# DerrickWang005/CRIS.pytorch

Hardware: AMD Instinct MI355X
Metric: train-step samples/sec, CRIS-R50 416x416 bs=64; loss parity vs ref (higher is better)
Workload: dtype bf16; 1 GPU; CRIS-R50 bf16 training step (fwd+BCE+bwd+Adam), 416x416, per-GPU bs=8, 17-token text, synthetic RefCOCO-shape batch resident in HBM (BASELINE.json configs[1]); global_batch=8, parallelism=dp1, launch=graph, graph_captured=True, syncbn_exchange=none, grad_exchange=none

## Files before the change

### cris/pytorch_amd/csrc/api.hip

```cpp
#include "common.h"
#include "../../../include/cris_hip.h"
#include <stdarg.h>
#include <string.h>

static thread_local char g_err[512] = {0};

void cris_set_error(const char* fmt, ...) {
    va_list ap;
    va_start(ap, fmt);
    vsnprintf(g_err, sizeof(g_err), fmt, ap);
    va_end(ap);
}

extern "C" const char* cris_last_error(void) { return g_err; }
extern "C" int cris_abi_version(void) { return CRIS_ABI_VERSION; }

extern "C" int cris_sizeof(const char* name) {
#define S(n) if (!strcmp(name, #n)) return (int)sizeof(n)
    S(cris_conv_gemm_params);
    S(cris_wgrad_params);
    S(cris_conv_gemm_group);
    S(cris_wgrad_group);
    S(cris_pack_desc);
    S(cris_conv_gemm_fp8_params);
    S(cris_pack_fp8_desc);
    S(cris_bn_apply_params);
    S(cris_bn_bwd_params);
    S(cris_ln_fwd_params);
    S(cris_ln_bwd_params);
    S(cris_sum_entry);
    S(cris_sum_group);
    S(cris_attn_params);
    S(cris_adam_desc);
    S(cris_ema_desc);
    S(cris_p2p_params);
    S(cris_p2p_link);
    S(cris_p2p_arena_params);
    S(cris_zero_ranges);
    S(cris_sample_desc);
    S(cris_eval_desc);
    S(cris_jpeg_info);
    S(cris_jpeg_image);
#undef S
    return -1;
}

extern "C" long cris_echo_conv_gemm(const void* vp) {
    const cris_conv_gemm_params* p = (const cris_conv_gemm_params*)vp;
    long h = 0;
    h = h * 31 + (long)(uintptr_t)p->A; h = h * 31 + (long)(uintptr_t)p->outT; h = h * 31 + p->T_sec_stride;
    h = h * 31 + p->lda; h = h * 31 + p->C; h = h * 31 + p->pad; h = h * 31 + p->ldb; h = h * 31 + p->K;
    h = h * 31 + p->act; h = h * 31 + p->out_f32; h = h * 31 + p->T_E; h = h * 31 + (long)(p->drop_p * 1000.f);
    h = h * 31 + p->drop_seed; h = h * 31 + p->drop_stream;
// ... 17 lines not shown
    const size_t tail0 = nvec * 16;
    if (blockIdx.x == 0 && tail0 + threadIdx.x < z.nbytes) reinterpret_cast<unsigned char*>(z.p)[tail0 + threadIdx.x] = 0;
}
extern "C" int cris_zero_many(const cris_zero_ranges* r, void* stream) {
    CRIS_CHECK_ARG(r && r->n > 0 && r->n <= CRIS_ZERO_RANGES_MAX, "1 .. CRIS_ZERO_RANGES_MAX ranges");
    size_t big = 0;
    for (int i = 0; i < r->n; ++i) {
        CRIS_CHECK_ARG(r->r[i].p && ((uintptr_t)r->r[i].p & 15) == 0, "ranges must be 16-byte aligned");
        if (r->r[i].nbytes > big) big = r->r[i].nbytes;
    }
    hipLaunchKernelGGL(zero_ranges_kernel, dim3(cris_grid_1d((long)(big / 16 + 1), 256, 2048), r->n), dim3(256), 0, (hipStream_t)stream, *r);
    CRIS_LAUNCH_CHECK();
    return 0;
}

extern "C" int cris_zero_bytes(void* p, size_t nbytes, void* stream) {
    if (!p || nbytes == 0) return 0;
    CRIS_CHECK_ARG(((uintptr_t)p & 15) == 0, "buffer must be 16-byte aligned");
    const size_t nvec = nbytes / 16;
    hipLaunchKernelGGL(zero_bytes_kernel, dim3(cris_grid_1d((long)(nvec ? nvec : 1), 256, 4096)), dim3(256), 0, (hipStream_t)stream,
                       (unsigned char*)p, nvec, nbytes);
    CRIS_LAUNCH_CHECK();
    return 0;
}
```

### cris/pytorch_amd/csrc/elementwise.hip

```cpp
#include <cmath>
#include "common.h"
#include "../../../include/cris_hip.h"

__device__ __forceinline__ void ld8f(const float* p, float* f) {
    const float4 a = *reinterpret_cast<const float4*>(p);
    const float4 b = *reinterpret_cast<const float4*>(p + 4);
    f[0] = a.x; f[1] = a.y; f[2] = a.z; f[3] = a.w; f[4] = b.x; f[5] = b.y; f[6] = b.z; f[7] = b.w;
}
__device__ __forceinline__ void ld8bf(const bf16_t* p, float* f) { unpack8(*reinterpret_cast<const uint4*>(p), f); }
__device__ __forceinline__ void st8bf(bf16_t* p, const float* f) { *reinterpret_cast<uint4*>(p) = pack8(f); }

#define GRID_STRIDE(idx, total) \
    for (long idx = (long)blockIdx.x * blockDim.x + threadIdx.x; idx < (total); idx += (long)gridDim.x * blockDim.x)

__global__ void stem_im2col_kernel(const float* __restrict__ img, int Bn, int H, int W, int OH, int OW, bf16_t* __restrict__ out) {
    const long total = (long)Bn * OH * OW * 4;
    const bool small = total < (1L << 24);
    GRID_STRIDE(idx, total) {
        const cris_idx4 q = cris_split4(idx, 4, OW, OH, small);
        const int kc = q.cv, ow = q.x, oh = q.y, b = q.b;
        const long m = idx >> 2;
        float v[8];
#pragma unroll
        for (int j = 0; j < 8; ++j) {
// ... 478 lines not shown
            float a = 0.f;
            for (int b = 0; b < Bn; ++b) a += dx[((size_t)b * L + r) * D + d];
            dpos[(size_t)r * D + d] = a;
        }
    }
}
extern "C" int cris_embed_bwd(const int64_t* tokens, const float* dx, int Bn, int L, int D, float* dtable, float* dpos,
                              unsigned char* row_live, void* stream) {
    CRIS_CHECK_ARG(tokens && dx && dtable && dpos, "bad args");
    hipLaunchKernelGGL(embed_bwd_kernel, dim3(cris_grid_1d((long)Bn * L * D, 256)), dim3(256), 0, (hipStream_t)stream, tokens, dx,
                       Bn, L, D, dtable, dpos, row_live);
    CRIS_LAUNCH_CHECK();
    return 0;
}

__global__ void eot_gather_kernel(const int64_t* tokens, const bf16_t* x, int L, int D, bf16_t* out, int* eot_index) {
    __shared__ int s_idx;
    const int b = blockIdx.x;
    if (threadIdx.x == 0) {
        int best = 0;
        int64_t bv = tokens[(size_t)b * L];
        for (int l = 1; l < L; ++l) {
            const int64_t v = tokens[(size_t)b * L + l];
            if (v > bv) { bv = v; best = l; }
        }
        s_idx = best;
        eot_index[b] = best;
    }
    __syncthreads();
    const bf16_t* src = x + ((size_t)b * L + s_idx) * D;
// ... 414 lines not shown
    CRIS_LAUNCH_CHECK();
    return 0;
}
extern "C" int cris_seg_loss_bwd(const float* logits, const float* target, int Bn, int HW, float w_bce, float w_dice, float pw, float s,
                                 const float* coef, const float* gscale, float* dlogits, void* stream) {
    CRIS_CHECK_ARG(logits && target && coef && dlogits, "null operand");
    CRIS_CHECK_ARG(Bn >= 1, "Bn must be >= 1");
    CRIS_CHECK_ARG(HW >= 1, "HW must be >= 1");
    if (seg_loss_check_config(__func__, w_bce, w_dice, pw, s)) return -1;
    hipLaunchKernelGGL(seg_loss_bwd_kernel, dim3(cris_grid_1d(HW, 256, 1024), Bn < SEG_MAX_GRID_Y ? Bn : SEG_MAX_GRID_Y), dim3(256), 0,
                       (hipStream_t)stream, logits, target, Bn, HW, w_bce, w_dice, pw, coef, gscale, dlogits);
    CRIS_LAUNCH_CHECK();
    return 0;
}

__global__ __launch_bounds__(1024) void train_metric_kernel(const float* x, const float* t, int Bn, int HW, float thr, float pr_iou, float* out) {
    __shared__ float si[16], su[16];
    float iou_sum = 0.f, pr_sum = 0.f;
    for (int b = 0; b < Bn; ++b) {
        float inter = 0.f, uni = 0.f;
        for (int i = threadIdx.x; i < HW; i += 1024) {
            const bool o = 1.f / (1.f + __expf(-x[(size_t)b * HW + i])) >= thr;
            const bool g = t[(size_t)b * HW + i] != 0.f;
            inter += (o && g) ? 1.f : 0.f;
            uni += (o || g) ? 1.f : 0.f;
        }
        inter = wave_sum(inter);
        uni = wave_sum(uni);
        __syncthreads();
        if ((threadIdx.x & 63) == 0) { si[threadIdx.x >> 6] = inter; su[threadIdx.x >> 6] = uni; }
        __syncthreads();
        if (threadIdx.x == 0) {
            float a = 0.f, u = 0.f;
#pragma unroll
            for (int w = 0; w < 16; ++w) { a += si[w]; u += su[w]; }
            const float iou = a / (u + 1e-6f);
            iou_sum += iou;
            pr_sum += iou > pr_iou ? 1.f : 0.f;
        }
    }
    if (threadIdx.x == 0) {
        out[0] = 100.f * iou_sum / (float)Bn;
        out[1] = 100.f * pr_sum / (float)Bn;
    }
}
extern "C" int cris_train_metric(const float* logits, const float* target, int Bn, int HW, float thr, float pr_iou, float* out,
                                 void* stream) {
    CRIS_CHECK_ARG(logits && target && out, "bad args");
    hipLaunchKernelGGL(train_metric_kernel, dim3(1), dim3(1024), 0, (hipStream_t)stream, logits, target, Bn, HW, thr, pr_iou, out);
    CRIS_LAUNCH_CHECK();
    return 0;
}

#define ADAM_ELEMS 8192
#define AP_T 64
#define AP_TN(PT) ((PT) == 9 ? 32 : 64)
#define AP_LROW(PT) (AP_T * (PT) + 2)

struct adam_coef {
    float beta1, beta2, eps, wd, bc1, rsb2, gscale;
    float keep;
};
__device__ __forceinline__ float adam_mul_rn(float a, float b) {
#pragma clang fp contract(off)
// ... 302 lines not shown
```

### cris/pytorch_amd/engine.py

```python
from __future__ import annotations

from typing import Callable, Dict, List, Optional

import torch
from torch import nn

from . import debug, ops, tables
from .arch import ClipSpec, HeadSpec, build_param_tree
from .ops import BF16, Drop, Geom, NO_DROP, pad8, pad32

F32 = torch.float32
BN_EPS, BN_MOM, LN_EPS = 1e-5, 0.1, 1e-5


class Act:
    __slots__ = ("t", "Bn", "H", "W", "C", "ld", "coff", "root", "_g", "aux")
    _engine = None

    def __init__(self, t, Bn, H, W, C, ld=None, coff=0, root=None):
        self.t, self.Bn, self.H, self.W, self.C = t, Bn, H, W, C
        self.ld = ld if ld is not None else C
        self.coff = coff
        self.root = root if root is not None else self
        self._g = None
# ... 62 lines not shown
        self.state_f32 = os.environ.get("CRIS_STATE_FP32", "0") == "1"
        self.P, self.Bf = params, buffers
        self.comm = comm or Comm()
        self.sync_bn = sync_bn and (self.comm.world > 1 or debug.HOOKS.force_dist)
        self.tape: List[Callable[[], None]] = []
        self.training = True
        self.seed = 0
        self.seed_dev = None
        self.loss_spec = None
        self.loss_terms = None
        self.side = torch.cuda.Stream(device=device) if torch.device(device).type == "cuda" else None
        if debug.HOOKS.no_side_stream:
            self.side = None
        self._wq, self._sq = ops.WgradQueue(self._flush_wgrads), ops.SumQueue()
        self._zslab, self._zcur, self._zneed, self._zneed_last = None, 0, 0, 0
        self._tables = {}
        self._build_grad_arena()
        self._build_packs()

    def gemm_layout(self, name):
        p = self.P[name]
        if name == "backbone.visual.conv1.weight":
            return p.shape[0], 27, 1, 32
        if p.dim() == 4:
            return p.shape[0], p.shape[1], p.shape[2] * p.shape[3], pad8(p.shape[1])
        return None

    def grad_param_layout(self, name):
        g, lay = self.G[name], self.gemm_layout(name)
        if lay is None or (lay[2] == 1 and lay[3] == lay[1]):
# ... 71 lines not shown
        self.grad_arena = torch.zeros(total, dtype=F32, device=self.dev)
        self.G = {name: self.grad_arena[o:o + n].view(shapes[name]) for name, (o, n) in offs.items()}
        self.grad_order = order
        self.grad_offsets = offs
        self.bn_pairs = pairs
        self.stage_ranges, zr = {}, {}
        for name in order:
            st = stage(name)
            lo, hi = offs[name][0], offs[name][0] + (offs[name][1] + 3) // 4 * 4
            a, b = self.stage_ranges.get(st, (lo, hi))
            self.stage_ranges[st] = (min(a, lo), max(b, hi))
            if needs_zero(name):
                a, b = zr.get(st, (lo, hi))
                zr[st] = (min(a, lo), max(b, hi))
        self.zero_ranges = [self.grad_arena[a:b] for a, b in sorted(zr.values())]

    def _add_pack(self, name, N, Cin, taps, Cpad=None, want_D=True, transposed=False):
        src = self.P[name]
        tab = self.packs[self.stage_of(name)]
        f, d = tab.add(src, N, Cin, taps, Cpad=Cpad, want_D=want_D, src_transposed=transposed)
        self.WF[name], self.WD[name] = f, d
        self.pack_info[name] = tab.info[-1]

    def _build_packs(self):
        self.packs = {st: ops.PackTable() for st in range(8)}
        self.packs_current = False
        self.WF, self.WD, self.pack_info = {}, {}, {}
        wd = not self.inference_only
        for name, p in self.P.items():
            if p.dim() == 4:
# ... 14 lines not shown
    def repack_stage(self, st):
        self.packs[st].run()

    def table(self, key, fn):
        if key not in self._tables:
            self._tables[key] = torch.from_numpy(fn()).to(self.dev)
        return self._tables[key]

    def _zero_slab_begin(self):
        need = self._zneed_last
        if need and (self._zslab is None or self._zslab.numel() < need):
            self._zslab = torch.empty(need, dtype=torch.uint8, device=self.dev)
        if self._zslab is not None:
            ops.zero_(self._zslab)
        self._zcur = self._zneed = 0

    def zeros(self, *shape, dtype=F32):
        n = dtype.itemsize
        for d in shape:
            n *= int(d)
        n_al = (n + 255) // 256 * 256
        self._zneed += n_al
        if n > 0 and self._zslab is not None and self._zcur + n_al <= self._zslab.numel():
            t = self._zslab[self._zcur:self._zcur + n].view(dtype).view(*shape)
            self._zcur += n_al
            return t
        return ops.zero_(torch.empty(*shape, dtype=dtype, device=self.dev))

    def empty(self, *shape, dtype=BF16):
        return torch.empty(*shape, dtype=dtype, device=self.dev)
# ... 208 lines not shown
                    dx, accum = dx_stream.grad_target()
                else:
                    dx, acc = x.grad_target()
                    accum = False
                    assert not acc, "bf16 LN input gradient cannot be accumulated"
                ops.ln_bwd(x.t, gamma, mean, rstd, rows, C, dx, ldx=x.ld, dy=None if (y is None or y.g is None) else y.g,
                           dypos=None if (ypos is None or ypos.g is None) else ypos.g,
                           dout_f32=None if outs is None else outs.g, dgamma=self.G[pfx + ".weight"], dbeta=self.G[pfx + ".bias"],
                           dx_accum=accum, in_relu=in_relu, in_drop=in_drop, out_drop=out_drop, queue=self._sq)

            self.tape.append(bwd)
        return y, ypos, outs

    def new_T(self, B, Hn, L, secs=1):
        Lpad = pad32(L)
        buf = self.zeros(secs, B * Hn * 64, Lpad, dtype=BF16)
        return dict(buf=buf, L=L, Lpad=Lpad, E=Hn * 64, sec_stride=B * Hn * 64 * Lpad)

    def attention(self, q: Act, k: Act, v: Act, Qt, Kt, Vt, B, Hn, Lq, Lk, *, causal=False, key_tokens=None, drop: Drop = NO_DROP):
        E = Hn * 64
        o = self.new_act(B, Lq, 1, E)
        lse = self.empty(B * Hn, Lq, dtype=F32)
        Lkp, Lqp = pad32(Lk), pad32(Lq)
        qv, kv, vv = q.t[:, q.coff:], k.t[:, k.coff:], v.t[:, v.coff:]
        prm = ops.attn_params(qv, kv, vv, Vt, B, Hn, Lq, Lk, Lkp, 64 ** -0.5, ldq=q.ld, ldk=k.ld, ldv=v.ld, Kt=Kt, Qt=Qt,
                              Lq_pad=Lqp, key_tokens=key_tokens, causal=causal, drop=drop)
        ops.attn_fwd(prm, o.t, lse, ldo=o.ld)
        if self.training:
            dOt = self.new_T(B, Hn, Lq)
            keep = (qv, kv, vv, Qt, Kt, Vt, key_tokens)

# ... 139 lines not shown
        if self.state_f32 and B <= ops.SMALL_MAX_ROWS:
            state = self._state_f32(word, x, xf, eot, B, L, D)
        else:
            rows = Act(self.empty(B, D), B, 1, 1, D)
            ops.eot_gather(word, xf.t, D, rows.t, eot)
            if self.training:
                def bwd_eot():
                    gx, acc = xf.grad_target()
                    if not acc:
                        ops.zero_(gx)
                    ops.eot_scatter_add(eot, rows.g, B, L, D, gx)
                self.tape.append(bwd_eot)
            state = self.gemm(rows, "backbone.text_projection", self.clip.embed_dim, w_transposed=True)
        if self.training:
            def bwd_embed():
                ops.embed_bwd(word, x0.g, self.G["backbone.token_embedding.weight"], self.G["backbone.positional_embedding"],
                              row_live=self.embed_live)
            self.tape.insert(self._text_tape_start, bwd_embed)
        return xf, state

    def _state_f32(self, word, x: Act, xf: Act, eot, B, L, D) -> Act:
        E = self.clip.embed_dim
        mean, rstd = xf.aux["ln_stats"]
        Pn = "backbone.text_projection"
        rows = torch.empty(B, D, dtype=F32, device=self.dev)
        ops.eot_gather_ln_f32(word, x.t, mean, rstd, self.P["backbone.ln_final.weight"], self.P["backbone.ln_final.bias"], D, rows, eot)
        state = Act(torch.empty(B, E, dtype=F32, device=self.dev), B, 1, 1, E)
        ops.linear_f32_small(rows, self.P[Pn], state.t, w_is_kn=True)
        if self.training:
            def bwd():
# ... 326 lines not shown
                ops.seg_loss_bwd(pred, msk, spec, coef, self._gscale, dpred)
            gx, acc = x.grad_target()
            assert not acc
            self._dwb = self.zeros(B, wb.ld)
            ops.dynconv_bwd(x.t, dpred, B, OH, OW, c, wb.t, gx, self._dwb)

        self.tape.append(bwd_loss)
        return pred, msk, loss.view(())

    def backward(self, gscale: Optional[torch.Tensor] = None, on_stage_done: Optional[Callable[[int], None]] = None):
        self._gscale = gscale
        Act._engine = self
        if debug.HOOKS.zero_all:
            ops.zero_(self.grad_arena)
        else:
            ops.zero_ranges(self.zero_ranges)
        marks = dict(self._stage_marks)
        (t0, t1), (v0, v1) = self._ranges["text"], self._ranges["visual"]
        head_start = max(t1, v1)
        def fire(i):
            if i in marks:
                self._flush_queues()
                if on_stage_done is not None:
                    for st in marks[i]:
                        on_stage_done(st)

        for i in range(len(self.tape) - 1, head_start - 1, -1):
            self.tape[i]()
            fire(i)
        self._flush_queues()
        if debug.HOOKS.hold_backward_fork:
# ... 32 lines not shown
```

### cris/pytorch_amd/hip.py

```python
import contextlib
import ctypes as C
import os

import torch

_HERE = os.path.dirname(os.path.abspath(__file__))
LIB_PATH = os.path.join(_HERE, "csrc", "libcris_hip.so")
if os.environ.get("CRIS_LIB_VARIANT"):
    LIB_PATH = os.path.join(_HERE, "csrc", "variants", "libcris_hip_%s.so" % os.environ["CRIS_LIB_VARIANT"])

P, I, L, F, U = C.c_void_p, C.c_int, C.c_long, C.c_float, C.c_uint32


class ConvGemmParams(C.Structure):
    _fields_ = [("A", P), ("Wt", P), ("bias", P), ("resid", P), ("out", P), ("outT", P), ("colsum", P), ("colsq", P),
                ("T_sec_stride", L),
                ("lda", I), ("a_coff", I),
                ("Bn", I), ("H", I), ("W", I), ("C", I),
                ("OH", I), ("OW", I), ("KH", I), ("KW", I), ("stride", I), ("pad", I),
                ("ldb", I),
                ("M", I), ("N", I), ("K", I),
                ("act", I),
                ("ldr", I), ("r_coff", I), ("resid_f32", I),
                ("ldc", I), ("c_coff", I), ("out_f32", I),
# ... 161 lines not shown
class EmaDesc(C.Structure):
    _fields_ = [("p", P), ("ema", P), ("n", L), ("row_live", P), ("row_len", I), ("block_start", I)]


ZERO_RANGES_MAX = 16


class ZeroRange(C.Structure):
    _fields_ = [("p", P), ("nbytes", C.c_size_t)]


class ZeroRanges(C.Structure):
    _fields_ = [("n", I), ("pad_", I), ("r", ZeroRange * ZERO_RANGES_MAX)]


class SampleDesc(C.Structure):
    _fields_ = [("img", P), ("mask", P), ("H", I), ("W", I), ("inv", C.c_double * 6)]


class EvalDesc(C.Structure):
    _fields_ = [("m", C.c_double * 6), ("w_out", I), ("h_out", I), ("map", I), ("row", I),
                ("mask_off", L), ("out_off", L), ("pitch", I), ("pad_", I)]


class JpegInfo(C.Structure):
    _fields_ = [("width", I), ("height", I), ("ncomp", I), ("hmax", I), ("vmax", I), ("mcus_x", I), ("mcus_y", I),
                ("restart_interval", I),
                ("comp_h", I * 3), ("comp_v", I * 3), ("blocks_w", I * 3), ("blocks_h", I * 3), ("down_w", I * 3), ("down_h", I * 3),
                ("quant", (C.c_ushort * 64) * 3),
                ("coef_offset", L * 3), ("coef_count", L), ("plane_offset", L * 3), ("plane_bytes", L), ("scan_offset", L),
# ... 15 lines not shown

class P2PLink(C.Structure):
    _fields_ = [("boxes", P), ("err", P), ("gen_dev", P),
                ("gen_host", I), ("rank", I), ("world", I),
                ("slot", I), ("slots", I), ("max_floats", I), ("spin_limit", I)]


class P2PArenaParams(C.Structure):
    _fields_ = [("arenas", P), ("lo", C.c_long), ("n", C.c_long), ("link", P2PLink), ("blocks", I)]


STRUCTS = {
    "cris_conv_gemm_params": ConvGemmParams, "cris_conv_gemm_group": ConvGemmGroup, "cris_wgrad_params": WgradParams, "cris_wgrad_group": WgradGroup, "cris_pack_desc": PackDesc,
    "cris_conv_gemm_fp8_params": ConvGemmFp8Params, "cris_pack_fp8_desc": PackFp8Desc,
    "cris_bn_apply_params": BnApplyParams, "cris_bn_bwd_params": BnBwdParams, "cris_ln_fwd_params": LnFwdParams,
    "cris_ln_bwd_params": LnBwdParams, "cris_sum_entry": SumEntry, "cris_sum_group": SumGroup, "cris_attn_params": AttnParams, "cris_adam_desc": AdamDesc, "cris_ema_desc": EmaDesc, "cris_p2p_params": P2PParams, "cris_p2p_link": P2PLink, "cris_p2p_arena_params": P2PArenaParams, "cris_zero_ranges": ZeroRanges,
    "cris_sample_desc": SampleDesc, "cris_eval_desc": EvalDesc, "cris_jpeg_info": JpegInfo, "cris_jpeg_image": JpegImage,
}

_SIGS = {
    "cris_last_error": (C.c_char_p, []),
    "cris_abi_version": (I, []),
    "cris_sizeof": (I, [C.c_char_p]),
    "cris_echo_conv_gemm": (L, [P]),
    "cris_conv_gemm": (I, [P, P]),
    "cris_conv_wgrad": (I, [P, P]),
    "cris_conv_wgrad_group": (I, [P, P]),
    "cris_conv_wgrad_tile": (I, [P]),
    "cris_wgrad_reduce": (I, [P, P]),
    "cris_wgrad_reduce_group": (I, [P, P]),
    "cris_wgrad_ws_floats": (L, [I, I, I, I]),
# ... 41 lines not shown
    "cris_fill_coords": (I, [P, I, I, I, I, I, I, P]),
    "cris_gather_samples_bf16": (I, [P, I, I, P, I, I, I, P, I, I, P]),
    "cris_add_bf16": (I, [P, I, I, P, I, I, P, I, I, I, I, P]),
    "cris_add_rowtable": (I, [P, I, P, I, P, I, I, I, P]),
    "cris_cast_f32_bf16": (I, [P, P, L, P]),
    "cris_cast_bf16_f32": (I, [P, P, L, I, P]),
    "cris_cast_f32_bf16_drop": (I, [P, P, L, F, U, U, U, P, P]),
    "cris_step_advance": (I, [P, P, P, P]),
    "cris_step_advance_micro": (I, [P, P, P, I, I, P]),
    "cris_axpy_f32": (I, [P, P, F, L, P]),
    "cris_grad_accumulate": (I, [P, P, L, I, P]),
    "cris_quickgelu_fwd": (I, [P, P, L, P]),
    "cris_quickgelu_bwd": (I, [P, P, P, L, P]),
    "cris_embed_fwd": (I, [P, P, P, I, I, I, P, P]),
    "cris_embed_bwd": (I, [P, P, I, I, I, P, P, P, P]),
    "cris_eot_gather": (I, [P, P, I, I, I, P, P, P]),
    "cris_eot_scatter_add": (I, [P, P, I, I, I, P, P]),
    "cris_eot_gather_ln_f32": (I, [P, P, P, P, P, P, I, I, I, P, P, P]),
    "cris_eot_scatter_add_f32": (I, [P, P, I, I, I, P, P]),
    "cris_linear_f32_small": (I, [P, I, P, I, I, P, I, I, I, P, I, I, P]),
    "cris_outer_sum_f32_small": (I, [P, I, P, I, I, I, I, P, I, P, P]),
    "cris_colstats_f32_small": (I, [P, I, I, I, P, P, P]),
    "cris_bn_relu_f32_small": (I, [P, I, P, P, I, I, P, I, P]),
    "cris_bn_relu_bwd_reduce_f32_small": (I, [P, I, P, I, P, P, P, P, I, I, P, P]),
    "cris_bn_relu_bwd_apply_f32_small": (I, [P, I, P, I, P, P, P, P, P, F, I, I, P, I, P]),
    "cris_posresize_fwd": (I, [P, P, I, I, I, P, P]),
    "cris_posresize_bwd": (I, [P, P, I, I, I, P, P]),
    "cris_batch_rowsum": (I, [P, I, I, I, I, P, P]),
    "cris_dynconv_fwd": (I, [P, I, I, I, I, P, I, P, P]),
    "cris_dynconv_bwd": (I, [P, P, I, I, I, I, P, I, P, P, P, P]),
    "cris_dynconv_bwd_ws_floats": (L, [I, I, I, I]),
    "cris_mask_resize_nearest": (I, [P, I, I, I, I, I, P, P]),
    "cris_bce_fwd": (I, [P, P, L, P, P, P]),
    "cris_bce_ws_floats": (I, []),
    "cris_bce_bwd": (I, [P, P, L, P, P, P]),
    "cris_seg_loss_fwd": (I, [P, P, I, I, F, F, F, F, P, P, P, P, P]),
    "cris_seg_loss_ws_floats": (L, [I]),
    "cris_seg_loss_bwd": (I, [P, P, I, I, F, F, F, F, P, P, P, P]),
    "cris_train_metric": (I, [P, P, I, I, F, F, P, P]),
    "cris_sigmoid_bicubic_up": (I, [P, I, I, I, I, I, P, P]),
    "cris_warp_affine_cubic": (I, [P, I, I, P, I, I, F, P, P]),
    "cris_threshold_iou": (I, [P, P, L, F, P, P]),
    "cris_eval_desc_fill": (I, [P, P, I, I, I, L, I, L, I]),
    "cris_eval_iou_batch": (I, [P, I, I, I, P, P, I, P, C.c_size_t, F, F, P, I, P, C.c_size_t, P]),
    "cris_predict_masks_batch": (I, [P, I, I, I, P, P, I, F, F, P, I, P, C.c_size_t, P]),
    "cris_preprocess_batch": (I, [P, I, I, I, P, P, P, P, P, P, P, P]),
    "cris_gray_sum_batch": (I, [P, P, I, P, P]),
    "cris_preprocess_batch_aug": (I, [P, I, I, I, P, P, P, P, P, P, P, P, P, P, P, P]),
    "cris_invert_affine": (I, [P, P]),
    "cris_remap_tables_u8": (I, [P, P]),
    "cris_zero_bytes": (I, [P, C.c_size_t, P]),
    "cris_zero_many": (I, [P, P]),
    "cris_adam_step": (I, [P, I, I, F, F, F, F, F, F, F, P, I, P]),
    "cris_adam_step_amp": (I, [P, I, I, F, F, F, F, F, F, F, P, P, P, I, P]),
    "cris_adamw_step": (I, [P, I, I, F, F, F, P, I, F, F, F, P, P, P, I, P]),
    "cris_counter_advance_unless": (I, [P, P, P]),
    "cris_adam_blocks": (I, [P]),
    "cris_adam_block_elems": (I, []),
    "cris_unpack_grads": (I, [P, I, I, P]),
    "cris_grad_sumsq": (I, [P, I, I, P, P]),
    "cris_grad_clip_finalize": (I, [P, I, F, F, P, P]),
    "cris_ema_blocks": (I, [P]),
    "cris_ema_advance": (I, [P, I, F, I, P, P]),
    "cris_ema_update": (I, [P, I, I, P, P]),
    "cris_adam_schedule_lrs": (I, [P, I, P, P, P, I, I, P, P]),
    "cris_p2p_mailbox_bytes": (C.c_size_t, [I, I, I]),
    "cris_p2p_alloc": (I, [C.c_size_t, P]),
# ... 119 lines not shown
```

### cris/pytorch_amd/ops.py

```python
from __future__ import annotations

import ctypes as C
import math
import os
from dataclasses import dataclass
from typing import Optional

import torch

from . import hip
from .hip import ptr

BF16 = torch.bfloat16


def _stream():
    return torch.cuda.current_stream().cuda_stream


def pad8(n: int) -> int:
    return (n + 7) // 8 * 8


def pad32(n: int) -> int:
# ... 696 lines not shown

def quickgelu_bwd(x, dy, dx):
    hip.call("cris_quickgelu_bwd", ptr(x), ptr(dy), ptr(dx), x.numel(), _stream())


def embed_fwd(tokens, table, pos, out):
    Bn, L = tokens.shape
    hip.call("cris_embed_fwd", ptr(tokens), ptr(table), ptr(pos), Bn, L, table.shape[1], ptr(out), _stream())


def embed_bwd(tokens, dx, dtable, dpos, row_live=None):
    Bn, L = tokens.shape
    hip.call("cris_embed_bwd", ptr(tokens), ptr(dx), Bn, L, dtable.shape[1], ptr(dtable), ptr(dpos), ptr(row_live), _stream())


def eot_gather(tokens, x, D, out, eot_index):
    Bn, L = tokens.shape
    hip.call("cris_eot_gather", ptr(tokens), ptr(x), Bn, L, D, ptr(out), ptr(eot_index), _stream())


def eot_scatter_add(eot_index, drows, Bn, L, D, dx):
    hip.call("cris_eot_scatter_add", ptr(eot_index), ptr(drows), Bn, L, D, ptr(dx), _stream())


SMALL_MAX_ROWS = 16


def eot_gather_ln_f32(tokens, x, mean, rstd, gamma, beta, D, out, eot_index):
    Bn, L = tokens.shape
    hip.call("cris_eot_gather_ln_f32", ptr(tokens), ptr(x), ptr(mean), ptr(rstd), ptr(gamma), ptr(beta), Bn, L, D, ptr(out), ptr(eot_index),
# ... 120 lines not shown


def seg_loss_fwd(logits, target, spec: SegLoss, loss, terms, coef):
    Bn = logits.shape[0]
    ws = torch.empty(hip.load().cris_seg_loss_ws_floats(Bn), dtype=torch.float32, device=logits.device)
    hip.call("cris_seg_loss_fwd", ptr(logits), ptr(target), Bn, logits.numel() // Bn, *spec.scalars, ptr(loss), ptr(terms), ptr(coef),
             ptr(ws), _stream())


def seg_loss_bwd(logits, target, spec: SegLoss, coef, gscale, dlogits):
    Bn = logits.shape[0]
    hip.call("cris_seg_loss_bwd", ptr(logits), ptr(target), Bn, logits.numel() // Bn, *spec.scalars, ptr(coef), ptr(gscale), ptr(dlogits),
             _stream())


def train_metric(logits, target, Bn, HW, out, thr=0.35, pr_iou=0.5):
    hip.call("cris_train_metric", ptr(logits), ptr(target), Bn, HW, float(thr), float(pr_iou), ptr(out), _stream())


def zero_(t):
    hip.call("cris_zero_bytes", ptr(t), t.numel() * t.element_size(), _stream())
    return t


def zero_ranges(tensors):
    for i in range(0, len(tensors), hip.ZERO_RANGES_MAX):
        chunk = tensors[i:i + hip.ZERO_RANGES_MAX]
        zr = hip.ZeroRanges()
        zr.n = len(chunk)
        for j, t in enumerate(chunk):
            zr.r[j].p, zr.r[j].nbytes = ptr(t), t.numel() * t.element_size()
        hip.call("cris_zero_many", C.byref(zr), _stream())


def torch_op(fn):
    fn()
    rec = hip.RECORDER
    if rec is not None:
        s = torch.cuda.current_stream()

        def run():
            if torch.cuda.current_stream() == s:
                fn()
            else:
                with torch.cuda.stream(s):
                    fn()
        rec.cmds.append((run, None, "torch_op"))
# ... 371 lines not shown
```

### cris/pytorch_amd/trainer.py

```python
import contextlib
import os
from typing import Optional

import torch

from . import capture, debug, ops
from .arch import ClipSpec, HeadSpec
from .engine import Engine


def strip_ddp_prefix(sd):
    keys = list(sd.keys())
    if keys and all(k.startswith("module.") for k in keys):
        return {k[len("module."):]: v for k, v in sd.items()}
    return sd


def split_state_dict(sd, device):
    sd = strip_ddp_prefix(sd)
    params = {k: v.to(device).contiguous() for k, v in sd.items()
              if v.is_floating_point() and not k.endswith(("running_mean", "running_var"))}
    buffers = {k: v.to(device).contiguous() for k, v in sd.items() if k.endswith(("running_mean", "running_var"))}
    return params, buffers

# ... 49 lines not shown
            for t in list(e.P.values()) + list(e.Bf.values()):
                self.comm.broadcast(t, 0)
        self._checked_batch = None
        names = [n for n in e.grad_order if n != "backbone.logit_scale"]
        self.names = names
        self.group = {n: (0 if in_backbone_group(n) else 1) for n in names}
        self.base_lr, self.lr_multi = base_lr, lr_multi
        self.weight_decay, self.decoupled_weight_decay, self.no_decay = decay_cfg
        self._no_decay_names = self._exempt(no_decay, [(n, e.P[n]) for n in names])
        if ((self.comm.world == 1 or getattr(self.comm, "supports_max_u8", False)) and self.weight_decays[EMBEDDING] == 0.0
                and os.environ.get("CRIS_ADAM_ROW_SKIP", "1") == "1" and torch.device(device).type == "cuda"):
            e.embed_live = torch.zeros(e.P["backbone.token_embedding.weight"].shape[0], dtype=torch.uint8, device=device)
        self._build_adam([base_lr] * len(names))
        self._apply_weight_decay()
        self.metric = torch.zeros(2, device=device)
        self.step_dev = torch.zeros(1, dtype=torch.int32, device=device)
        self.seed_dev = torch.zeros(1, dtype=torch.int32, device=device)
        self.xgen_dev = torch.zeros(1, dtype=torch.int32, device=device)
        self.syncbn_exchange = "none" if not e.sync_bn else "collective"
        if (e.sync_bn and os.environ.get("CRIS_SYNCBN_P2P", "1") == "1"
                and torch.device(device).type == "cuda" and hasattr(self.comm, "enable_p2p")):
            cmax = max(e.P[pfx + ".weight"].numel() for pfx in e.bn_prefixes)
            why = self.comm.enable_p2p(slots=2 * len(e.bn_prefixes) + 8, max_floats=4 * cmax, gen_dev=self.xgen_dev)
            if why is None:
                fused = getattr(self.comm, "_fused", False)
                self.syncbn_exchange = "p2p mailboxes, exchanged inside the BatchNorm launches" if fused else "p2p mailboxes, one exchange kernel per BatchNorm"
            else:
                self.syncbn_exchange = "collective (mailboxes refused: %s)" % why
        self.grad_exchange = "none" if (self.comm.world == 1 and not debug.HOOKS.force_dist) else "rccl"
        if (os.environ.get("CRIS_GRAD_EXCHANGE", "rccl") == "p2p" and getattr(self.comm, "p2p", None) is not None
# ... 58 lines not shown
        return float(max_norm)

    def _invalidate(self):
        self._graph = self._cmds = None
        self._eager_steps = 0

    def set_accum_steps(self, accum_steps):
        self.accum_steps = checked_int("accum_steps", accum_steps, 1)
        if self.accum_steps > 1:
            if self._acc is None:
                self._acc = torch.empty_like(self.engine.grad_arena)
                self._loss_acc = torch.zeros((), device=self.device)
                self._metric_micro = torch.zeros(2, device=self.device)
        else:
            self._acc = self._loss_acc = self._metric_micro = None
        self._size_terms_acc()
        self._invalidate()

    def set_loss(self, spec):
        self.engine.set_loss(spec)
        self._size_terms_acc()
        self._invalidate()

    def _size_terms_acc(self):
        if self.engine.loss_spec is not None and self.accum_steps > 1:
            if self._terms_acc is None:
                self._terms_acc = torch.zeros(2, device=self.device)
        else:
            self._terms_acc = None

# ... 127 lines not shown
                ops.axpy_f32(self._loss_acc, loss, 1.0 / K)
                if self._terms_acc is not None:
                    ops.axpy_f32(self._terms_acc, e.loss_terms, 1.0 / K)
            self._metric(pred, msk)
            e.backward(on_stage_done=self._stage_hook(m))
        if self._exchanges():
            ops.torch_op(self.comm.wait_all)
        self._update(1.0 / (self.comm.world * K))
        return (loss if K == 1 else self._loss_acc), pred, msk

    def _exchanges(self):
        return self.comm.world > 1 or debug.HOOKS.force_dist

    def _metric(self, pred, msk):
        e, K = self.engine, self.accum_steps
        if e.side is not None:
            cur = torch.cuda.current_stream()
            ops.torch_op(lambda: e.side.wait_stream(cur))
        with (torch.cuda.stream(e.side) if e.side is not None else contextlib.nullcontext()):
            ops.train_metric(pred, msk, pred.shape[0], pred.shape[2] * pred.shape[3], self.metric if K == 1 else self._metric_micro)
            if K > 1:
                ops.axpy_f32(self.metric, self._metric_micro, 1.0 / K)

    def _stage_hook(self, m):
        e, K, exchange = self.engine, self.accum_steps, self._exchanges()
        if K == 1 and not exchange:
            return None
        last = m == K - 1

        def on_stage(st):
            lo, hi = e.stage_ranges[st]
            g = e.grad_arena[lo:hi]
            if K > 1:
                acc = self._acc[lo:hi]
                if not last:
# ... 172 lines not shown
```

### include/cris_hip.h

```cpp
#ifndef CRIS_HIP_H
#define CRIS_HIP_H
#include <stddef.h>
#include <stdint.h>
#ifdef __cplusplus
extern "C" {
#endif

typedef uint16_t cris_bf16;

const char* cris_last_error(void);
#define CRIS_ABI_VERSION 8
int cris_abi_version(void);
int cris_sizeof(const char* struct_name);
long cris_echo_conv_gemm(const void* conv_gemm_params);

typedef struct {
    const cris_bf16* A;
    const cris_bf16* Wt;
    const float* bias;
    const void* resid;
    void* out;
    cris_bf16* outT;
    float* colsum;
    float* colsq;
// ... 254 lines not shown
                      int C, void* stream);
int cris_cast_f32_bf16(const float* x, cris_bf16* y, long n, void* stream);
int cris_cast_bf16_f32(const cris_bf16* x, float* y, long n, int accum, void* stream);
int cris_cast_f32_bf16_drop(const float* x, cris_bf16* y, long n, float drop_p, uint32_t drop_thresh, uint32_t seed,
                            uint32_t stream_id, const uint32_t* seed_dev, void* stream);
int cris_step_advance(int32_t* step, uint32_t* seed, int32_t* exchange_gen, void* stream);
int cris_step_advance_micro(int32_t* step, uint32_t* seed, int32_t* exchange_gen, int micro, int accum, void* stream);
int cris_axpy_f32(float* dst, const float* src, float alpha, long n, void* stream);
int cris_grad_accumulate(float* dst, const float* src, long n, int mode, void* stream);
int cris_quickgelu_fwd(const cris_bf16* x, cris_bf16* y, long n, void* stream);
int cris_quickgelu_bwd(const cris_bf16* x, const cris_bf16* dy, cris_bf16* dx, long n, void* stream);
int cris_embed_fwd(const int64_t* tokens, const float* table, const float* pos, int Bn, int L, int D, float* out,
                   void* stream);
int cris_embed_bwd(const int64_t* tokens, const float* dx, int Bn, int L, int D, float* dtable, float* dpos, unsigned char* row_live,
                   void* stream);
int cris_eot_gather(const int64_t* tokens, const cris_bf16* x, int Bn, int L, int D, cris_bf16* out, int* eot_index,
                    void* stream);
int cris_eot_scatter_add(const int* eot_index, const cris_bf16* dstate_rows, int Bn, int L, int D, cris_bf16* dx,
                         void* stream);
int cris_posresize_fwd(const float* R, const float* pos, int T, int G, int C, float* posr, void* stream);
int cris_posresize_bwd(const float* R, const float* dposr, int T, int G, int C, float* dpos, void* stream);
int cris_batch_rowsum(const cris_bf16* dx, int ldx, int Bn, int T, int C, float* out, void* stream);
int cris_dynconv_fwd(const cris_bf16* x, int Bn, int H, int W, int C, const float* wb, int ldwb, float* pred,
                     void* stream);
int cris_dynconv_bwd(const cris_bf16* x, const float* dpred, int Bn, int H, int W, int C, const float* wb, int ldwb,
                     cris_bf16* dx, float* dwb, float* ws, void* stream);
long cris_dynconv_bwd_ws_floats(int Bn, int H, int W, int ldwb);
int cris_mask_resize_nearest(const float* mask, int Bn, int IH, int IW, int OH, int OW, float* out, void* stream);
int cris_bce_fwd(const float* logits, const float* target, long n, float* loss, float* ws, void* stream);
int cris_bce_ws_floats(void);
int cris_bce_bwd(const float* logits, const float* target, long n, const float* gscale, float* dlogits, void* stream);
int cris_seg_loss_fwd(const float* logits, const float* target, int Bn, int HW, float w_bce, float w_dice, float pw, float s,
                      float* loss, float* terms, float* coef, float* ws, void* stream);
long cris_seg_loss_ws_floats(int Bn);
int cris_seg_loss_bwd(const float* logits, const float* target, int Bn, int HW, float w_bce, float w_dice, float pw, float s,
                      const float* coef, const float* gscale, float* dlogits, void* stream);
int cris_train_metric(const float* logits, const float* target, int Bn, int HW, float thr, float pr_iou, float* out,
                      void* stream);
int cris_sigmoid_bicubic_up(const float* logits, int Bn, int h, int w, int H, int W, float* out, void* stream);
int cris_warp_affine_cubic(const float* src, int H, int W, const double* mat, int w_out, int h_out, float border, float* dst,
                           void* stream);
int cris_threshold_iou(const float* pred, const float* mask, long n, float thr, int* counts, void* stream);
typedef struct {
    double m[6];
    int w_out, h_out;
    int map, row;
    long mask_off, out_off;
    int pitch, pad_;
} cris_eval_desc;
int cris_eval_desc_fill(cris_eval_desc* desc, const double* mat, int w_out, int h_out, int map, long mask_off, int pitch,
                        long out_off, int row);
int cris_eval_iou_batch(const float* probs, int P, int H, int W, const cris_eval_desc* descs_host, const cris_eval_desc* descs_dev,
                        int n, const unsigned char* masks, size_t mask_bytes, float thr, float border, int* counts, int count_rows,
// ... 12 lines not shown
                          const float* lut_img, const float* lut_mask, const unsigned char* border_rgb ,
                          float* img_out, float* mask_out, void* stream);
int cris_gray_sum_batch(const cris_sample_desc* samples_host, const cris_sample_desc* samples_dev, int n, unsigned long long* sums_dev,
                        void* stream);
int cris_preprocess_batch_aug(const cris_sample_desc* samples_dev, int n, int S_h, int S_w, const short* tab_linear, const short* tab_cubic,
                              const float* lut_img, const float* lut_mask, const unsigned char* border_rgb ,
                              const float* factors_dev, const unsigned long long* sums_dev, const float* unit_dev,
                              const float* norm , float* img_out, float* mask_out, void* stream);
int cris_invert_affine(const double* mat, double* inv);
int cris_remap_tables_u8(short* tab_linear, short* tab_cubic);
int cris_zero_bytes(void* p, size_t nbytes, void* stream);
#define CRIS_ZERO_RANGES_MAX 16
typedef struct { void* p; size_t nbytes; } cris_zero_range;
typedef struct { int n; int pad_; cris_zero_range r[CRIS_ZERO_RANGES_MAX]; } cris_zero_ranges;
int cris_zero_many(const cris_zero_ranges* r, void* stream);

typedef struct {
    float* p; const float* g; float* m; float* v;
    long n;
    float lr; float pad_;
    int block_start; int taps;
    int cin; int cpad;
    cris_bf16* dstF; cris_bf16* dstD;
    int N; int npad;
    int transposed; int ldF;
    const unsigned char* row_live;
    int row_len; int ldD;
} cris_adam_desc;
int cris_adam_step(const cris_adam_desc* dev_table, int n_desc, int total_blocks, float beta1, float beta2, float eps,
                   float weight_decay, float bias_corr1, float bias_corr2, float grad_scale, const int32_t* step_dev,
// ... 139 lines not shown
```

Measured before the change: 681.6 samples/s.

## Skip dense zeroing of embedding grad, pool attention T buffers, parallelize train metric

Three separate changes cut redundant work in the training step. First, the token-embedding gradient table is dropped from the per-step dense zero ranges. Instead, only the rows touched by earlier steps are re-zeroed, using a ring of recorded token ids. Second, the padded attention transpose buffers are pooled across steps, and only their pad tail columns are zeroed rather than the whole slab. Third, the train-metric kernel moves from a single block to one block per sample, with a last-block atomic reduction. Together these remove bulk memset traffic and a serialized reduction, at the cost of stateful buffers whose correctness depends on the slot and ring logic.

```diff
diff --git a/cris/pytorch_amd/csrc/api.hip b/cris/pytorch_amd/csrc/api.hip
--- a/cris/pytorch_amd/csrc/api.hip
+++ b/cris/pytorch_amd/csrc/api.hip
@@ -37,6 +37,7 @@
     S(cris_p2p_link);
     S(cris_p2p_arena_params);
     S(cris_zero_ranges);
+    S(cris_zero_tails);
     S(cris_sample_desc);
     S(cris_eval_desc);
     S(cris_jpeg_info);
@@ -84,6 +85,45 @@
     return 0;
 }
 
+#define ZT_WORDS 1024
+__device__ __host__ static inline int zero_tail_words(const cris_zero_tail& z) { return z.rows * ((z.ld - (z.col0 & ~1)) >> 1); }
+__global__ __launch_bounds__(256) void zero_tails_kernel(const cris_zero_tails t) {
+    int blk = blockIdx.x, i = 0;
+    for (; i < t.n; ++i) {
+        const int nb = (zero_tail_words(t.t[i]) + ZT_WORDS - 1) / ZT_WORDS;
+        if (blk < nb) break;
+        blk -= nb;
+    }
+    if (i == t.n) return;
+    const cris_zero_tail z = t.t[i];
+    const int c0 = z.col0 & ~1;
+    const int nw = (z.ld - c0) >> 1, total = z.rows * nw;
+    for (int w = blk * ZT_WORDS + threadIdx.x; w < total && w < (blk + 1) * ZT_WORDS; w += 256) {
+        const int row = w / nw;
+        const int col = c0 + 2 * (w - row * nw);
+        unsigned short* q = reinterpret_cast<unsigned short*>(z.p) + (size_t)row * z.ld + col;
+        if (col < z.col0) q[1] = 0;
+        else *reinterpret_cast<unsigned*>(q) = 0u;
+    }
+}
+extern "C" int cris_zero_tails_bf16(const cris_zero_tails* t, void* stream) {
+    CRIS_CHECK_ARG(t && t->n > 0 && t->n <= CRIS_ZERO_TAILS_MAX, "1 .. CRIS_ZERO_TAILS_MAX matrices");
+    long blocks = 0;
+    for (int i = 0; i < t->n; ++i) {
+        const cris_zero_tail& z = t->t[i];
+        CRIS_CHECK_ARG(z.p && ((uintptr_t)z.p & 3) == 0, "matrices must be 4-byte aligned");
+        CRIS_CHECK_ARG(z.rows >= 1 && z.ld >= 2 && (z.ld & 1) == 0, "rows >= 1 and an even ld");
+        CRIS_CHECK_ARG(z.col0 >= 0 && z.col0 <= z.ld && z.ld - z.col0 <= CRIS_ZERO_TAIL_COLS, "col0 must be within CRIS_ZERO_TAIL_COLS of ld");
+        CRIS_CHECK_ARG(z.rows <= (1 << 26), "rows must be <= 2^26");
+        blocks += (zero_tail_words(z) + ZT_WORDS - 1) / ZT_WORDS;
+    }
+    if (blocks == 0) return 0;
+    CRIS_CHECK_ARG(blocks < (1L << 31), "too many rows");
+    hipLaunchKernelGGL(zero_tails_kernel, dim3((unsigned)blocks), dim3(256), 0, (hipStream_t)stream, *t);
+    CRIS_LAUNCH_CHECK();
+    return 0;
+}
+
 extern "C" int cris_zero_bytes(void* p, size_t nbytes, void* stream) {
     if (!p || nbytes == 0) return 0;
     CRIS_CHECK_ARG(((uintptr_t)p & 15) == 0, "buffer must be 16-byte aligned");
diff --git a/cris/pytorch_amd/csrc/elementwise.hip b/cris/pytorch_amd/csrc/elementwise.hip
--- a/cris/pytorch_amd/csrc/elementwise.hip
+++ b/cris/pytorch_amd/csrc/elementwise.hip
@@ -516,6 +516,30 @@
     return 0;
 }
 
+__global__ __launch_bounds__(1024) void embed_rezero_kernel(int64_t* ids, int n_slots, int cap, int slot, const int64_t* tokens, int R, int D,
+                                                            int vocab, float* dtable) {
+    const int DV = D >> 2, lane = threadIdx.x & 63;
+    for (int r = threadIdx.x >> 6; r < n_slots * cap; r += 16) {
+        const int64_t tok = ids[r];
+        if (tok < 0 || tok >= vocab) continue;
+        float4* row = reinterpret_cast<float4*>(dtable + (size_t)tok * D);
+        for (int dv = lane; dv < DV; dv += 64) row[dv] = make_float4(0.f, 0.f, 0.f, 0.f);
+    }
+    __syncthreads();
+    for (int r = threadIdx.x; r < cap; r += 1024) ids[(size_t)slot * cap + r] = r < R ? tokens[r] : -1;
+}
+extern "C" int cris_embed_rezero(int64_t* ids, int n_slots, int cap, int slot, const int64_t* tokens, int R, int D, int vocab,
+                                 float* dtable, void* stream) {
+    CRIS_CHECK_ARG(ids && tokens && dtable, "null operand");
+    CRIS_CHECK_ARG(n_slots >= 1 && slot >= 0 && slot < n_slots, "slot must be in [0, n_slots)");
+    CRIS_CHECK_ARG(R >= 1 && R <= cap, "R must be in [1, cap]");
+    CRIS_CHECK_ARG(D >= 4 && !(D & 3) && vocab >= 1, "D must be a multiple of 4, vocab >= 1");
+    CRIS_CHECK_ARG(((uintptr_t)dtable & 15) == 0, "dtable must be 16-byte aligned");
+    hipLaunchKernelGGL(embed_rezero_kernel, dim3(1), dim3(1024), 0, (hipStream_t)stream, ids, n_slots, cap, slot, tokens, R, D, vocab, dtable);
+    CRIS_LAUNCH_CHECK();
+    return 0;
+}
+
 __global__ void eot_gather_kernel(const int64_t* tokens, const bf16_t* x, int L, int D, bf16_t* out, int* eot_index) {
     __shared__ int s_idx;
     const int b = blockIdx.x;
@@ -960,10 +984,11 @@
     return 0;
 }
 
-__global__ __launch_bounds__(1024) void train_metric_kernel(const float* x, const float* t, int Bn, int HW, float thr, float pr_iou, float* out) {
+__global__ __launch_bounds__(1024) void train_metric_kernel(const float* x, const float* t, int Bn, int HW, float thr, float pr_iou, float* out,
+                                                            unsigned* ws) {
     __shared__ float si[16], su[16];
     float iou_sum = 0.f, pr_sum = 0.f;
-    for (int b = 0; b < Bn; ++b) {
+    for (int b = blockIdx.x; b < Bn; b += gridDim.x) {
         float inter = 0.f, uni = 0.f;
         for (int i = threadIdx.x; i < HW; i += 1024) {
             const bool o = 1.f / (1.f + __expf(-x[(size_t)b * HW + i])) >= thr;
@@ -981,19 +1006,41 @@
 #pragma unroll
             for (int w = 0; w < 16; ++w) { a += si[w]; u += su[w]; }
             const float iou = a / (u + 1e-6f);
+            if (ws) {
+                __hip_atomic_store(ws + 1 + b, __float_as_uint(iou), __ATOMIC_RELAXED, __HIP_MEMORY_SCOPE_AGENT);
+            } else {
+                iou_sum += iou;
+                pr_sum += iou > pr_iou ? 1.f : 0.f;
+            }
+        }
+    }
+    if (threadIdx.x != 0) return;
+    if (ws) {
+        if (__hip_atomic_fetch_add(ws, 1u, __ATOMIC_ACQ_REL, __HIP_MEMORY_SCOPE_AGENT) != gridDim.x - 1) return;
+        for (int b = 0; b < Bn; ++b) {
+            const float iou = __uint_as_float(__hip_atomic_load(ws + 1 + b, __ATOMIC_RELAXED, __HIP_MEMORY_SCOPE_AGENT));
             iou_sum += iou;
             pr_sum += iou > pr_iou ? 1.f : 0.f;
         }
-    }
-    if (threadIdx.x == 0) {
-        out[0] = 100.f * iou_sum / (float)Bn;
-        out[1] = 100.f * pr_sum / (float)Bn;
-    }
+        __hip_atomic_store(ws, 0u, __ATOMIC_RELAXED, __HIP_MEMORY_SCOPE_AGENT);
+    }
+    out[0] = 100.f * iou_sum / (float)Bn;
+    out[1] = 100.f * pr_sum / (float)Bn;
 }
 extern "C" int cris_train_metric(const float* logits, const float* target, int Bn, int HW, float thr, float pr_iou, float* out,
                                  void* stream) {
     CRIS_CHECK_ARG(logits && target && out, "bad args");
-    hipLaunchKernelGGL(train_metric_kernel, dim3(1), dim3(1024), 0, (hipStream_t)stream, logits, target, Bn, HW, thr, pr_iou, out);
+    hipLaunchKernelGGL(train_metric_kernel, dim3(1), dim3(1024), 0, (hipStream_t)stream, logits, target, Bn, HW, thr, pr_iou, out, nullptr);
+    CRIS_LAUNCH_CHECK();
+    return 0;
+}
+extern "C" int cris_train_metric_blocks(const float* logits, const float* target, int Bn, int HW, float thr, float pr_iou, float* out,
+                                        unsigned* ws, void* stream) {
+    CRIS_CHECK_ARG(logits && target && out && ws, "null operand");
+    CRIS_CHECK_ARG(Bn >= 1, "Bn must be >= 1");
+    CRIS_CHECK_ARG(HW >= 1, "HW must be >= 1");
+    hipLaunchKernelGGL(train_metric_kernel, dim3(Bn < 256 ? Bn : 256), dim3(1024), 0, (hipStream_t)stream, logits, target, Bn, HW, thr,
+                       pr_iou, out, ws);
     CRIS_LAUNCH_CHECK();
     return 0;
 }
diff --git a/cris/pytorch_amd/engine.py b/cris/pytorch_amd/engine.py
--- a/cris/pytorch_amd/engine.py
+++ b/cris/pytorch_amd/engine.py
@@ -100,6 +100,8 @@
             self.side = None
         self._wq, self._sq = ops.WgradQueue(self._flush_wgrads), ops.SumQueue()
         self._zslab, self._zcur, self._zneed, self._zneed_last = None, 0, 0, 0
+        self._tpool, self._tused = {}, {}
+        self._embed_ids, self._embed_slot = None, 0
         self._tables = {}
         self._build_grad_arena()
         self._build_packs()
@@ -201,6 +203,16 @@
                 a, b = zr.get(st, (lo, hi))
                 zr[st] = (min(a, lo), max(b, hi))
         self.zero_ranges = [self.grad_arena[a:b] for a, b in sorted(zr.values())]
+        e0, en = offs["backbone.token_embedding.weight"]
+        e1 = e0 + (en + 3) // 4 * 4
+        self._zero_ranges_sparse = [self.grad_arena[a:b] for lo, hi in sorted(zr.values())
+                                    for a, b in (((lo, e0), (e1, hi)) if lo <= e0 and e1 <= hi else ((lo, hi),)) if b > a]
+
+    def embed_rows_sparse(self, slots, cap=256):
+        self._embed_ids = None
+        if slots:
+            ops.zero_(self.G["backbone.token_embedding.weight"])
+            self._embed_ids = torch.full((slots, cap), -1, dtype=torch.int64, device=self.dev)
 
     def _add_pack(self, name, N, Cin, taps, Cpad=None, want_D=True, transposed=False):
         src = self.P[name]
@@ -245,6 +257,8 @@
         if self._zslab is not None:
             ops.zero_(self._zslab)
         self._zcur = self._zneed = 0
+        ops.zero_tails([(t.view(-1, t.shape[-1]), key[2]) for key, bufs in self._tpool.items() for t in bufs])
+        self._tused = {}
 
     def zeros(self, *shape, dtype=F32):
         n = dtype.itemsize
@@ -483,7 +497,12 @@
 
     def new_T(self, B, Hn, L, secs=1):
         Lpad = pad32(L)
-        buf = self.zeros(secs, B * Hn * 64, Lpad, dtype=BF16)
+        key = (secs, B * Hn * 64, L)
+        bufs, k = self._tpool.setdefault(key, []), self._tused.get(key, 0)
+        self._tused[key] = k + 1
+        if k == len(bufs):
+            bufs.append(ops.zero_(torch.empty(secs, B * Hn * 64, Lpad, dtype=BF16, device=self.dev)))
+        buf = bufs[k]
         return dict(buf=buf, L=L, Lpad=Lpad, E=Hn * 64, sec_stride=B * Hn * 64 * Lpad)
 
     def attention(self, q: Act, k: Act, v: Act, Qt, Kt, Vt, B, Hn, Lq, Lk, *, causal=False, key_tokens=None, drop: Drop = NO_DROP):
@@ -653,6 +672,12 @@
             state = self.gemm(rows, "backbone.text_projection", self.clip.embed_dim, w_transposed=True)
         if self.training:
             def bwd_embed():
+                if self._embed_ids is not None:
+                    if self._embed_ids.shape[1] < B * L:
+                        self.embed_rows_sparse(self._embed_ids.shape[0], cap=B * L)
+                    ops.embed_rezero(self._embed_ids, self._embed_slot % self._embed_ids.shape[0], word,
+                                     self.G["backbone.token_embedding.weight"])
+                    self._embed_slot += 1
                 ops.embed_bwd(word, x0.g, self.G["backbone.token_embedding.weight"], self.G["backbone.positional_embedding"],
                               row_live=self.embed_live)
             self.tape.insert(self._text_tape_start, bwd_embed)
@@ -1009,7 +1034,7 @@
         if debug.HOOKS.zero_all:
             ops.zero_(self.grad_arena)
         else:
-            ops.zero_ranges(self.zero_ranges)
+            ops.zero_ranges(self.zero_ranges if self._embed_ids is None else self._zero_ranges_sparse)
         marks = dict(self._stage_marks)
         (t0, t1), (v0, v1) = self._ranges["text"], self._ranges["visual"]
         head_start = max(t1, v1)
diff --git a/cris/pytorch_amd/hip.py b/cris/pytorch_amd/hip.py
--- a/cris/pytorch_amd/hip.py
+++ b/cris/pytorch_amd/hip.py
@@ -199,6 +199,18 @@
     _fields_ = [("n", I), ("pad_", I), ("r", ZeroRange * ZERO_RANGES_MAX)]
 
 
+ZERO_TAILS_MAX = 64
+ZERO_TAIL_COLS = 32
+
+
+class ZeroTail(C.Structure):
+    _fields_ = [("p", P), ("rows", I), ("ld", I), ("col0", I), ("pad_", I)]
+
+
+class ZeroTails(C.Structure):
+    _fields_ = [("n", I), ("pad_", I), ("t", ZeroTail * ZERO_TAILS_MAX)]
+
+
 class SampleDesc(C.Structure):
     _fields_ = [("img", P), ("mask", P), ("H", I), ("W", I), ("inv", C.c_double * 6)]
 
@@ -244,7 +256,7 @@
     "cris_conv_gemm_params": ConvGemmParams, "cris_conv_gemm_group": ConvGemmGroup, "cris_wgrad_params": WgradParams, "cris_wgrad_group": WgradGroup, "cris_pack_desc": PackDesc,
     "cris_conv_gemm_fp8_params": ConvGemmFp8Params, "cris_pack_fp8_desc": PackFp8Desc,
     "cris_bn_apply_params": BnApplyParams, "cris_bn_bwd_params": BnBwdParams, "cris_ln_fwd_params": LnFwdParams,
-    "cris_ln_bwd_params": LnBwdParams, "cris_sum_entry": SumEntry, "cris_sum_group": SumGroup, "cris_attn_params": AttnParams, "cris_adam_desc": AdamDesc, "cris_ema_desc": EmaDesc, "cris_p2p_params": P2PParams, "cris_p2p_link": P2PLink, "cris_p2p_arena_params": P2PArenaParams, "cris_zero_ranges": ZeroRanges,
+    "cris_ln_bwd_params": LnBwdParams, "cris_sum_entry": SumEntry, "cris_sum_group": SumGroup, "cris_attn_params": AttnParams, "cris_adam_desc": AdamDesc, "cris_ema_desc": EmaDesc, "cris_p2p_params": P2PParams, "cris_p2p_link": P2PLink, "cris_p2p_arena_params": P2PArenaParams, "cris_zero_ranges": ZeroRanges, "cris_zero_tails": ZeroTails,
     "cris_sample_desc": SampleDesc, "cris_eval_desc": EvalDesc, "cris_jpeg_info": JpegInfo, "cris_jpeg_image": JpegImage,
 }
 
@@ -316,6 +328,7 @@
     "cris_quickgelu_bwd": (I, [P, P, P, L, P]),
     "cris_embed_fwd": (I, [P, P, P, I, I, I, P, P]),
     "cris_embed_bwd": (I, [P, P, I, I, I, P, P, P, P]),
+    "cris_embed_rezero": (I, [P, I, I, I, P, I, I, I, P, P]),
     "cris_eot_gather": (I, [P, P, I, I, I, P, P, P]),
     "cris_eot_scatter_add": (I, [P, P, I, I, I, P, P]),
     "cris_eot_gather_ln_f32": (I, [P, P, P, P, P, P, I, I, I, P, P, P]),
@@ -340,6 +353,7 @@
     "cris_seg_loss_ws_floats": (L, [I]),
     "cris_seg_loss_bwd": (I, [P, P, I, I, F, F, F, F, P, P, P, P]),
     "cris_train_metric": (I, [P, P, I, I, F, F, P, P]),
+    "cris_train_metric_blocks": (I, [P, P, I, I, F, F, P, P, P]),
     "cris_sigmoid_bicubic_up": (I, [P, I, I, I, I, I, P, P]),
     "cris_warp_affine_cubic": (I, [P, I, I, P, I, I, F, P, P]),
     "cris_threshold_iou": (I, [P, P, L, F, P, P]),
@@ -353,6 +367,7 @@
     "cris_remap_tables_u8": (I, [P, P]),
     "cris_zero_bytes": (I, [P, C.c_size_t, P]),
     "cris_zero_many": (I, [P, P]),
+    "cris_zero_tails_bf16": (I, [P, P]),
     "cris_adam_step": (I, [P, I, I, F, F, F, F, F, F, F, P, I, P]),
     "cris_adam_step_amp": (I, [P, I, I, F, F, F, F, F, F, F, P, P, P, I, P]),
     "cris_adamw_step": (I, [P, I, I, F, F, F, P, I, F, F, F, P, P, P, I, P]),
diff --git a/cris/pytorch_amd/ops.py b/cris/pytorch_amd/ops.py
--- a/cris/pytorch_amd/ops.py
+++ b/cris/pytorch_amd/ops.py
@@ -734,6 +734,12 @@
     hip.call("cris_embed_bwd", ptr(tokens), ptr(dx), Bn, L, dtable.shape[1], ptr(dtable), ptr(dpos), ptr(row_live), _stream())
 
 
+def embed_rezero(ids, slot, tokens, dtable):
+    assert ids.dtype == torch.int64 and ids.dim() == 2 and ids.is_contiguous() and tokens.is_contiguous()
+    hip.call("cris_embed_rezero", ptr(ids), ids.shape[0], ids.shape[1], slot, ptr(tokens), tokens.numel(), dtable.shape[1],
+             dtable.shape[0], ptr(dtable), _stream())
+
+
 def eot_gather(tokens, x, D, out, eot_index):
     Bn, L = tokens.shape
     hip.call("cris_eot_gather", ptr(tokens), ptr(x), Bn, L, D, ptr(out), ptr(eot_index), _stream())
@@ -884,8 +890,12 @@
              _stream())
 
 
-def train_metric(logits, target, Bn, HW, out, thr=0.35, pr_iou=0.5):
-    hip.call("cris_train_metric", ptr(logits), ptr(target), Bn, HW, float(thr), float(pr_iou), ptr(out), _stream())
+def train_metric(logits, target, Bn, HW, out, thr=0.35, pr_iou=0.5, ws=None):
+    if ws is None:
+        hip.call("cris_train_metric", ptr(logits), ptr(target), Bn, HW, float(thr), float(pr_iou), ptr(out), _stream())
+        return
+    assert ws.dtype == torch.int32 and ws.numel() >= Bn + 1
+    hip.call("cris_train_metric_blocks", ptr(logits), ptr(target), Bn, HW, float(thr), float(pr_iou), ptr(out), ptr(ws), _stream())
 
 
 def zero_(t):
@@ -901,6 +911,18 @@
         for j, t in enumerate(chunk):
             zr.r[j].p, zr.r[j].nbytes = ptr(t), t.numel() * t.element_size()
         hip.call("cris_zero_many", C.byref(zr), _stream())
+
+
+def zero_tails(mats):
+    mats = [(t, c) for t, c in mats if c < t.shape[1]]
+    for i in range(0, len(mats), hip.ZERO_TAILS_MAX):
+        chunk = mats[i:i + hip.ZERO_TAILS_MAX]
+        zt = hip.ZeroTails()
+        zt.n = len(chunk)
+        for j, (t, c) in enumerate(chunk):
+            assert t.dtype == BF16 and t.dim() == 2 and t.is_contiguous()
+            zt.t[j].p, zt.t[j].rows, zt.t[j].ld, zt.t[j].col0 = ptr(t), t.shape[0], t.shape[1], c
+        hip.call("cris_zero_tails_bf16", C.byref(zt), _stream())
 
 
 def torch_op(fn):
diff --git a/cris/pytorch_amd/trainer.py b/cris/pytorch_amd/trainer.py
--- a/cris/pytorch_amd/trainer.py
+++ b/cris/pytorch_amd/trainer.py
@@ -87,6 +87,7 @@
         self._build_adam([base_lr] * len(names))
         self._apply_weight_decay()
         self.metric = torch.zeros(2, device=device)
+        self._metric_ws = torch.zeros(65, dtype=torch.int32, device=device)
         self.step_dev = torch.zeros(1, dtype=torch.int32, device=device)
         self.seed_dev = torch.zeros(1, dtype=torch.int32, device=device)
         self.xgen_dev = torch.zeros(1, dtype=torch.int32, device=device)
@@ -175,6 +176,8 @@
                 self._metric_micro = torch.zeros(2, device=self.device)
         else:
             self._acc = self._loss_acc = self._metric_micro = None
+        if torch.device(self.device).type == "cuda":
+            self.engine.embed_rows_sparse(self.accum_steps if self.comm.world == 1 else 0)
         self._size_terms_acc()
         self._invalidate()
 
@@ -332,11 +335,14 @@
 
     def _metric(self, pred, msk):
         e, K = self.engine, self.accum_steps
+        if self._metric_ws.numel() < pred.shape[0] + 1:
+            self._metric_ws = torch.zeros(pred.shape[0] + 1, dtype=torch.int32, device=self.device)
         if e.side is not None:
             cur = torch.cuda.current_stream()
             ops.torch_op(lambda: e.side.wait_stream(cur))
         with (torch.cuda.stream(e.side) if e.side is not None else contextlib.nullcontext()):
-            ops.train_metric(pred, msk, pred.shape[0], pred.shape[2] * pred.shape[3], self.metric if K == 1 else self._metric_micro)
+            ops.train_metric(pred, msk, pred.shape[0], pred.shape[2] * pred.shape[3], self.metric if K == 1 else self._metric_micro,
+                             ws=self._metric_ws)
             if K > 1:
                 ops.axpy_f32(self.metric, self._metric_micro, 1.0 / K)
 
diff --git a/include/cris_hip.h b/include/cris_hip.h
--- a/include/cris_hip.h
+++ b/include/cris_hip.h
@@ -292,6 +292,8 @@
                    void* stream);
 int cris_embed_bwd(const int64_t* tokens, const float* dx, int Bn, int L, int D, float* dtable, float* dpos, unsigned char* row_live,
                    void* stream);
+int cris_embed_rezero(int64_t* ids, int n_slots, int cap, int slot, const int64_t* tokens, int R, int D, int vocab, float* dtable,
+                      void* stream);
 int cris_eot_gather(const int64_t* tokens, const cris_bf16* x, int Bn, int L, int D, cris_bf16* out, int* eot_index,
                     void* stream);
 int cris_eot_scatter_add(const int* eot_index, const cris_bf16* dstate_rows, int Bn, int L, int D, cris_bf16* dx,
@@ -315,6 +317,8 @@
                       const float* coef, const float* gscale, float* dlogits, void* stream);
 int cris_train_metric(const float* logits, const float* target, int Bn, int HW, float thr, float pr_iou, float* out,
                       void* stream);
+int cris_train_metric_blocks(const float* logits, const float* target, int Bn, int HW, float thr, float pr_iou, float* out,
+                             unsigned* ws, void* stream);
 int cris_sigmoid_bicubic_up(const float* logits, int Bn, int h, int w, int H, int W, float* out, void* stream);
 int cris_warp_affine_cubic(const float* src, int H, int W, const double* mat, int w_out, int h_out, float border, float* dst,
                            void* stream);
@@ -357,6 +361,11 @@
 typedef struct { void* p; size_t nbytes; } cris_zero_range;
 typedef struct { int n; int pad_; cris_zero_range r[CRIS_ZERO_RANGES_MAX]; } cris_zero_ranges;
 int cris_zero_many(const cris_zero_ranges* r, void* stream);
+#define CRIS_ZERO_TAILS_MAX 64
+#define CRIS_ZERO_TAIL_COLS 32
+typedef struct { void* p; int rows; int ld; int col0; int pad_; } cris_zero_tail;
+typedef struct { int n; int pad_; cris_zero_tail t[CRIS_ZERO_TAILS_MAX]; } cris_zero_tails;
+int cris_zero_tails_bf16(const cris_zero_tails* t, void* stream);
 
 typedef struct {
     float* p; const float* g; float* m; float* v;
```

New measurement: 682.6 samples/s, median of 3. No clear change (+0.1%).
